# manuelbb-upb/Morbit.jl

Hardware: AMD Instinct MI355X
Metric: RBF build+solve+eval cycles/sec (higher is better)
Workload: dtype f64

## Files before the change

### morbit.jl_amd/csrc/common.hpp

```cpp
#pragma once
#include <hip/hip_runtime.h>
#include <rocblas/rocblas.h>
#include <rocsolver/rocsolver.h>

#include <cmath>
#include <cstdlib>
#include <cstdint>
#include <cstdio>
#include <cstring>
#include <map>
#include <string>
#include <vector>

#include "../../include/mrbf.h"
#include "descent_problem.hpp"
#include "model_pool.hpp"

namespace mrbf {

struct KP {
    int kid;
    double a, b;
    double a2;
    double sgn;
// ... 154 lines not shown
int input_fetch(mrbf_ctx *ctx, const double *src, size_t count, double *dst);
int input_view(mrbf_ctx *ctx, const double *user, size_t count, double *&arena, const double **dev);
int output_put(mrbf_ctx *ctx, double *dst, const double *src, size_t count);
int fetch_linear_rows(mrbf_ctx *ctx, const mrbf_ps_problem *prob, int d, double *A, double *b);
descent::Shape descent_shape(const mrbf_ps_problem *prob, const mrbf_model *const *models, int64_t n_starts,
                             std::vector<descent::SlotShape> &slots);
void pin_reset(mrbf_ctx *ctx);
void pin_flush(mrbf_ctx *ctx);
void pin_discard(mrbf_ctx *ctx);
char *pin_take(mrbf_ctx *ctx, size_t bytes);
struct PinGuard {
    mrbf_ctx *ctx;
    bool flushed = false;
    explicit PinGuard(mrbf_ctx *c) : ctx(c) { pin_reset(c); }
    void flush() {
        pin_flush(ctx);
        flushed = true;
    }
    ~PinGuard() {
        if (!flushed) pin_discard(ctx);
    }
    PinGuard(const PinGuard &) = delete;
    PinGuard &operator=(const PinGuard &) = delete;
};
enum HpinSlot : int {
    HPIN_FIT_FLAGS = 0,
    HPIN_FIT_SCAL = 4,
    HPIN_SMALL_FLAGS = 8,
    HPIN_SMALL_SCAL = 12,
    HPIN_SMALL_CHK = 16,
    HPIN_RESIDUAL = 20,
    HPIN_R4_COUNT = 24,
    HPIN_MEGA_STAT = 63,
};

inline int64_t round_up(int64_t x, int64_t m) { return (x + m - 1) / m * m; }

inline const char *mrbf_env(const char *name) {
    const char *gate = std::getenv("MRBF_EXPERIMENTS");
    if (!gate || std::atoi(gate) == 0) return nullptr;
    return std::getenv(name);
}

int launch_center_pad(mrbf_ctx *ctx, const double *X, int64_t n, int d, const double *mean_or_null, double *mean_out,
                      double *Xc, int64_t npad, int dpad, double *sq);
int launch_poly_matrix(mrbf_ctx *ctx, const double *C, int64_t n, int d, int q, double *Pi, int64_t ldpi);
int launch_transpose(mrbf_ctx *ctx, const double *in, int64_t rows, int64_t cols, double *out);
int launch_gram(mrbf_ctx *ctx, int mode, const double *C, const double *Xc, const double *sq, int64_t n, int64_t npad,
                int d, int dpad, const KP &kp, double *Phi, int64_t ld);
int launch_cross_gram(mrbf_ctx *ctx, const double *X, int64_t m, const double *C, int64_t n, int d, const KP &kp, double *K);
bool gram_w_applies(const mrbf_ctx *ctx, const mrbf_model *M);
int launch_gram_w(mrbf_ctx *ctx, const mrbf_model *M, double *Phi, int64_t ld, double **Wpart_out, double **rspart_out, int *nseg_out);
int launch_projection_small(mrbf_ctx *ctx, const mrbf_model *M, const double *Wpart, const double *rspart, int nseg, const double *linv,
                            const double *Q1, double *W1, double *G, double *scal, int *flags, int K2, int skip, double *PA, double *PB,
                            double *v0);
int eval_model(mrbf_ctx *ctx, const mrbf_model *M, int64_t m, const double *Xdev, double *vals_dev, double *jac_dev,
               mrbf_eval_info *info, EvalHints hints = {});
int potrf_blocked_tall(mrbf_ctx *ctx, int64_t ncols, int64_t mrows, double *A, int64_t lda, int *dinfo, double *linv_all, PotrfOpts opt = {});
int potrf_mega_tall(mrbf_ctx *ctx, int64_t ncols, int64_t mrows, double *A, int64_t lda, int *dinfo, double *linv_all, PotrfOpts opt = {});
mega::Knobs mega_knobs_from_env();
int potrf_lower(mrbf_ctx *ctx, int impl, int64_t n, double *A, int64_t lda, int *info_host);
int fit_model(mrbf_ctx *ctx, mrbf_model *M, const double *Ydev, mrbf_fit_info *info);
int build_model_shell(mrbf_ctx *ctx, int64_t n, int d, int k, const double *Cdev, int kid, double a, double b, int deg,
                      mrbf_model **out);
void destroy_model(mrbf_ctx *ctx, mrbf_model *M);
void model_set_dims(mrbf_model *M, int64_t n, int d, int k, int kid, double a, double b, int deg);
size_t model_block_layout(const mrbf_model *M, size_t off[7]);
void model_carve(mrbf_model *M, char *base, const size_t off[7]);
int model_block_acquire(mrbf_ctx *ctx, size_t total, void **p, size_t *bytes);
void model_block_release(mrbf_ctx *ctx, void *p, size_t bytes, bool slab = false);
int fit_check(mrbf_ctx *ctx, mrbf_model *M, const double *Y, mrbf_fit_info *info);
int mega_collect_stat(mrbf_ctx *ctx);
int mega_stat_enqueue(mrbf_ctx *ctx);
int mega_stat_finish(mrbf_ctx *ctx);

}
```

### morbit.jl_amd/csrc/gram_fused.hip

```cpp
#include "radial.hpp"

namespace mrbf {

typedef double v4d __attribute__((ext_vector_type(4)));
typedef double v2d __attribute__((ext_vector_type(2)));

constexpr int GW_LDT = 66;

template <int KID, bool FAST>
__global__ __launch_bounds__(256, 2) void gram_w_kernel(const double *__restrict__ Xc, const double *__restrict__ sq, int64_t n,
                                                        int64_t npad, double *__restrict__ Phi, int64_t ld, KP p, int nt, int nseg,
                                                        int seglen, double *__restrict__ Wpart, double *__restrict__ rspart, int dbg) {
    __shared__ __attribute__((aligned(16))) double T[2][64 * GW_LDT];
    __shared__ double Tsq[2][64];
    const int tid = threadIdx.x, lane = tid & 63, wave = tid >> 6;
    const int l15 = lane & 15, l4 = lane >> 4;
    const int seg = blockIdx.x % nseg, I = nt - 1 - (int)(blockIdx.x / nseg);
    const int jt0 = seg * seglen;
    const int jt1 = (jt0 + seglen < nt) ? jt0 + seglen : nt;
    const int64_t iw0 = (int64_t)I * 128 + 32 * wave;
    double bI[2][16];
#pragma unroll
    for (int it = 0; it < 2; ++it)
#pragma unroll
// ... 146 lines not shown
        }
    }
#pragma unroll
    for (int tt = 0; tt < 4; ++tt)
#pragma unroll
        for (int r = 0; r < 4; ++r) {
            const int t = tt * 16 + l4 + 4 * r;
#pragma unroll
            for (int it = 0; it < 2; ++it) Wpart[((int64_t)seg * 64 + t) * npad + iw0 + it * 16 + l15] = wacc[tt][it][r];
        }
#pragma unroll
    for (int it = 0; it < 2; ++it) {
        double x = rs[it];
        x += __shfl_xor(x, 16);
        x += __shfl_xor(x, 32);
        if (l4 == 0) rspart[(int64_t)seg * npad + iw0 + it * 16 + l15] = x;
    }
}

__device__ __forceinline__ double sum_partials(const double *__restrict__ p, int cnt, int64_t stride) {
    double sp[8] = {0.0, 0.0, 0.0, 0.0, 0.0, 0.0, 0.0, 0.0};
    int c = 0;
    for (; c + 32 <= cnt; c += 32) {
        double v[32];
#pragma unroll
        for (int u = 0; u < 32; ++u) v[u] = p[(int64_t)(c + u) * stride];
#pragma unroll
        for (int u = 0; u < 32; ++u) sp[u & 7] += v[u];
    }
    for (; c + 8 <= cnt; c += 8) {
        double v[8];
#pragma unroll
        for (int u = 0; u < 8; ++u) v[u] = p[(int64_t)(c + u) * stride];
#pragma unroll
        for (int u = 0; u < 8; ++u) sp[u] += v[u];
    }
    for (int u = 0; c + u < cnt; ++u) sp[u] += p[(int64_t)(c + u) * stride];
    return ((sp[0] + sp[1]) + (sp[2] + sp[3])) + ((sp[4] + sp[5]) + (sp[6] + sp[7]));
}

constexpr int PJ_LS = 68;
constexpr int PJ_QP = 80;

__device__ __forceinline__ v4d pj_tile(const double *As, const double *Bs, int mt, int nt, int K, int l15, int l4) {
    v4d acc = {0.0, 0.0, 0.0, 0.0};
    const double *ap = As + (mt * 16 + l15) * PJ_LS + l4;
    const double *bp = Bs + (nt * 16 + l15) * PJ_LS + l4;
    for (int k = 0; k < K; k += 4) acc = __builtin_amdgcn_mfma_f64_16x16x4f64(ap[k], bp[k], acc, 0, 0, 0);
    return acc;
}

__global__ __launch_bounds__(256) void proj_reduce_kernel(const double *__restrict__ Wpart, const double *__restrict__ rspart, int nseg,
                                                          int64_t npad, int64_t n, int d, int q, const double *__restrict__ linv,
                                                          const double *__restrict__ Q1, double rsqrtn, double *__restrict__ W1,
                                                          double *__restrict__ Gp, double *__restrict__ trp) {
    __shared__ double Ws[64 * PJ_LS];
    __shared__ double Ls[64 * PJ_LS];
    __shared__ double W1s[PJ_QP * PJ_LS];
    __shared__ double Qs[PJ_QP * PJ_LS];
    const int tid = threadIdx.x, i = tid & 63, g = tid >> 6;
    const int lane = tid & 63, wave = tid >> 6, l15 = lane & 15, l4 = lane >> 4;
    const int64_t R0 = (int64_t)blockIdx.x * 64;
    const bool live = R0 + i < n;
    constexpr int Q4 = PJ_QP / 4;
    double qv[Q4];
#pragma unroll
    for (int u = 0; u < Q4; ++u) {
        const int a = g + 4 * u;
        qv[u] = (a < q && live) ? Q1[R0 + i + (int64_t)a * npad] : 0.0;
    }
    const double rsv = (g == 0 && live) ? sum_partials(rspart + R0 + i, nseg, npad) * rsqrtn : 0.0;
    if (q > 1) {
        double lv[16];
#pragma unroll
        for (int u = 0; u < 16; ++u) {
            const int e = tid + 256 * u, c = e & 63, t = e >> 6;
            lv[u] = (c < d && t <= c) ? linv[c + (int64_t)t * 128] : 0.0;
        }
#pragma unroll
        for (int half = 0; half < 2; ++half) {
            double sv[8] = {0.0, 0.0, 0.0, 0.0, 0.0, 0.0, 0.0, 0.0};
            for (int s0 = 0; s0 < nseg; s0 += 8) {
                double wv[8][8];
#pragma unroll
                for (int u = 0; u < 8; ++u)
#pragma unroll
                    for (int sgm = 0; sgm < 8; ++sgm) {
                        const int t = g * 16 + half * 8 + u;
                        wv[u][sgm] = s0 + sgm < nseg ? Wpart[((int64_t)(s0 + sgm) * 64 + t) * npad + R0 + i] : 0.0;
                    }
#pragma unroll
                for (int u = 0; u < 8; ++u)
                    sv[u] += ((wv[u][0] + wv[u][1]) + (wv[u][2] + wv[u][3])) + ((wv[u][4] + wv[u][5]) + (wv[u][6] + wv[u][7]));
            }
#pragma unroll
            for (int u = 0; u < 8; ++u) Ws[i * PJ_LS + (g * 16 + half * 8 + u)] = live ? sv[u] : 0.0;
        }
#pragma unroll
        for (int u = 0; u < 16; ++u) {
            const int e = tid + 256 * u;
            Ls[(e & 63) * PJ_LS + (e >> 6)] = lv[u];
        }
    }
#pragma unroll
    for (int u = 0; u < Q4; ++u) {
        const int a = g + 4 * u;
        Qs[a * PJ_LS + i] = qv[u];
        if (a > d || q == 1) W1s[a * PJ_LS + i] = 0.0;
    }
    if (g == 0) {
        W1s[i] = rsv;
        W1[R0 + i] = rsv;
    }
    __syncthreads();
    if (q > 1) {
#pragma unroll 1
        for (int tile = wave; tile < 16; tile += 4) {
            const int ct = tile >> 2, it = tile & 3;
            const v4d acc = pj_tile(Ls, Ws, ct, it, 64, l15, l4);
#pragma unroll
            for (int r = 0; r < 4; ++r) {
                const int c = ct * 16 + l4 + 4 * r, ii = it * 16 + l15;
                if (c < d) {
                    W1s[(1 + c) * PJ_LS + ii] = acc[r];
                    W1[R0 + ii + (int64_t)(1 + c) * npad] = acc[r];
                }
            }
        }
    }
    __syncthreads();
    double *out = Gp + (size_t)blockIdx.x * q * q;
    const int qt = (q + 15) >> 4;
#pragma unroll 1
    for (int tile = wave; tile < qt * qt; tile += 4) {
        const int at = tile % qt, bt = tile / qt;
        const v4d acc = pj_tile(Qs, W1s, at, bt, 64, l15, l4);
#pragma unroll
        for (int r = 0; r < 4; ++r) {
            const int a = at * 16 + l4 + 4 * r, bb = bt * 16 + l15;
            if (a < q && bb < q) out[a + bb * q] = acc[r];
            if (at == bt && a == bb && a < q) Ls[a] = acc[r];
        }
    }
    __syncthreads();
    if (tid == 0) {
        double tr = 0.0;
        for (int a = 0; a < q; ++a) tr += Ls[a];
        trp[blockIdx.x] = tr;
    }
}

__global__ __launch_bounds__(256) void proj_shift_kernel(const double *__restrict__ Gp, const double *__restrict__ trp, int nchunks, int q,
                                                         double nphi0, double nmq, double *__restrict__ G, double *__restrict__ Mh,
                                                         double *__restrict__ scal, int *__restrict__ flags) {
    __shared__ double dg[256];
    __shared__ double smu;
    const int tid = threadIdx.x;
    const size_t qq = (size_t)q * q;
    const int idx = blockIdx.x * 256 + tid;
    const double *p0 = Gp + (idx < (int)qq ? idx : 0);
    double tv = 0.0;
    for (int c = tid; c < nchunks; c += 256) tv += trp[c];
    double s0[8] = {0, 0, 0, 0, 0, 0, 0, 0};
    int c = 0;
    for (; c + 64 <= nchunks; c += 64) {
        double v0[64];
#pragma unroll
        for (int u = 0; u < 64; ++u) v0[u] = p0[(size_t)(c + u) * qq];
#pragma unroll
        for (int u = 0; u < 64; ++u) s0[u & 7] += v0[u];
    }
    for (; c < nchunks; ++c) s0[c & 7] += p0[(size_t)c * qq];
    const double gv = ((s0[0] + s0[1]) + (s0[2] + s0[3])) + ((s0[4] + s0[5]) + (s0[6] + s0[7]));
    dg[tid] = tv;
    __syncthreads();
    for (int w = 128; w > 0; w >>= 1) {
        if (tid < w) dg[tid] += dg[tid + w];
        __syncthreads();
    }
    if (tid == 0) {
        const double tr = dg[0];
        const double mu = (nphi0 - tr) / nmq;
        const bool ok = mu > 0.0 && mu < 1e300;
        smu = ok ? mu : 1.0;
        if (blockIdx.x == 0) {
            scal[0] = tr;
            scal[1] = smu;
            flags[2] = ok ? 0 : 1;
        }
    }
    __syncthreads();
    if (idx < (int)qq) {
        G[idx] = gv;
        Mh[idx] = 0.5 * gv + ((idx % q) == (idx / q) ? 0.5 * smu : 0.0);
    }
}

__global__ __launch_bounds__(256) void proj_panels_kernel(const double *__restrict__ Q1, const double *__restrict__ W1,
                                                          const double *__restrict__ Mh, int64_t n, int64_t npad, int q, int K2, int skip,
                                                          double *__restrict__ PA, double *__restrict__ PB, double *__restrict__ v0) {
    __shared__ double Qs[64 * PJ_LS];
    __shared__ double Ms[PJ_QP * PJ_LS];
    const int tid = threadIdx.x, i = tid & 63, g = tid >> 6;
    const int lane = tid & 63, wave = tid >> 6, l15 = lane & 15, l4 = lane >> 4;
    const int64_t R0 = (int64_t)blockIdx.x * 64;
    const bool live = R0 + i < n;
    constexpr int QA = 17;
    double qv[QA];
#pragma unroll
    for (int u = 0; u < QA; ++u) {
        const int a = g + 4 * u;
        qv[u] = (a < q && live) ? Q1[R0 + i + (int64_t)a * npad] : 0.0;
    }
    constexpr int ME = (PJ_QP * PJ_LS + 255) / 256;
    double mv[ME];
#pragma unroll
    for (int u = 0; u < ME; ++u) {
        const int e = tid + 256 * u, bb = e / PJ_LS, a = e % PJ_LS;
        mv[u] = (a < q && bb < q) ? Mh[a + bb * q] : 0.0;
    }
#pragma unroll
    for (int u = 0; u < ME; ++u) {
        const int e = tid + 256 * u;
        if (e < PJ_QP * PJ_LS) Ms[e] = mv[u];
    }
#pragma unroll
    for (int u = 0; u < QA; ++u) Qs[i * PJ_LS + g + 4 * u] = qv[u];
    __syncthreads();
    const int qq = q - skip, qt = (q + 15) >> 4, K = (q + 3) & ~3;
#pragma unroll 1
    for (int tile = wave; tile < qt * 4; tile += 4) {
        const int bt = tile >> 2, it = tile & 3;
        const v4d acc = pj_tile(Ms, Qs, bt, it, K, l15, l4);
        const int ii = it * 16 + l15;
        const bool lv = R0 + ii < n;
        double w1[4], qb[4];
#pragma unroll
        for (int r = 0; r < 4; ++r) {
            const int b = bt * 16 + l4 + 4 * r;
            w1[r] = (b < q && lv) ? W1[R0 + ii + (int64_t)b * npad] : 0.0;
            qb[r] = b < q ? Qs[ii * PJ_LS + b] : 0.0;
        }
#pragma unroll
        for (int r = 0; r < 4; ++r) {
            const int b = bt * 16 + l4 + 4 * r;
            if (b >= q) continue;
            const double v = lv ? w1[r] - acc[r] : 0.0;
            if (b >= skip) {
                const int c = b - skip;
                PA[R0 + ii + (int64_t)c * npad] = qb[r];
                PB[R0 + ii + (int64_t)c * npad] = v;
                PA[R0 + ii + (int64_t)(qq + c) * npad] = v;
                PB[R0 + ii + (int64_t)(qq + c) * npad] = qb[r];
            } else {
                v0[R0 + ii] = v;
            }
        }
    }
    for (int c = 2 * qq + g; c < K2; c += 4) {
        PA[R0 + i + (int64_t)c * npad] = 0.0;
        PB[R0 + i + (int64_t)c * npad] = 0.0;
    }
}

bool gram_w_applies(const mrbf_ctx *ctx, const mrbf_model *M) {
    static const int on = mrbf_env("MRBF_GRAM_FUSED") ? atoi(mrbf_env("MRBF_GRAM_FUSED")) : 1;
    if (!on || ctx->gram_mode != 0) return false;
    if (M->dpad != 64 || M->q < 1 || M->q > 65 || M->n < 1024) return false;
    return M->kp.fast || M->kp.kid == MRBF_GAUSSIAN || M->kp.kid == MRBF_THIN_PLATE_SPLINE;
}

int launch_gram_w(mrbf_ctx *ctx, const mrbf_model *M, double *Phi, int64_t ld, double **Wpart_out, double **rspart_out, int *nseg_out) {
    const int nt = (int)(M->npad / 128);
    static const int dbg = mrbf_env("MRBF_GW_DBG") ? atoi(mrbf_env("MRBF_GW_DBG")) : 0;
    static const int wgs = mrbf_env("MRBF_GW_WGS") ? atoi(mrbf_env("MRBF_GW_WGS")) : 512;
    int nseg = wgs / nt;
    if (nseg < 1) nseg = 1;
    if (nseg > nt) nseg = nt;
    const int seglen = (nt + nseg - 1) / nseg;
    nseg = (nt + seglen - 1) / seglen;
    double *Wpart, *rspart;
    MRBF_TRY(get_buf(ctx, S_GW_PART, (size_t)nseg * 64 * M->npad, &Wpart));
    MRBF_TRY(get_buf(ctx, S_GW_RS, (size_t)nseg * M->npad, &rspart));
    const dim3 grid((unsigned)(nt * nseg));
    if (M->kp.fast) {
        MRBF_DISPATCH_KID(M->kp.kid, hipLaunchKernelGGL((gram_w_kernel<KID, true>), grid, dim3(256), 0, ctx->stream, M->Xc, M->sq, M->n,
                                                        M->npad, Phi, ld, M->kp, nt, nseg, seglen, Wpart, rspart, dbg));
    } else if (M->kp.kid == MRBF_GAUSSIAN) {
        hipLaunchKernelGGL((gram_w_kernel<MRBF_GAUSSIAN, false>), grid, dim3(256), 0, ctx->stream, M->Xc, M->sq, M->n, M->npad, Phi, ld,
                           M->kp, nt, nseg, seglen, Wpart, rspart, dbg);
    } else {
        hipLaunchKernelGGL((gram_w_kernel<MRBF_THIN_PLATE_SPLINE, false>), grid, dim3(256), 0, ctx->stream, M->Xc, M->sq, M->n, M->npad,
                           Phi, ld, M->kp, nt, nseg, seglen, Wpart, rspart, dbg);
    }
    MRBF_HIP(ctx, hipGetLastError());
    *Wpart_out = Wpart;
    *rspart_out = rspart;
    *nseg_out = nseg;
    return 0;
}

int launch_projection_small(mrbf_ctx *ctx, const mrbf_model *M, const double *Wpart, const double *rspart, int nseg, const double *linv,
                            const double *Q1, double *W1, double *G, double *scal, int *flags, int K2, int skip, double *PA, double *PB,
                            double *v0) {
    const int64_t n = M->n, npad = M->npad;
    const int q = M->q, nch = (int)(npad / 64);
    double *Gp, *Mh;
    MRBF_TRY(get_buf(ctx, S_GW_GP, (size_t)nch * q * q + nch, &Gp));
    MRBF_TRY(get_buf(ctx, S_GW_M, (size_t)q * q, &Mh));
    double *trp = Gp + (size_t)nch * q * q;
    hipLaunchKernelGGL(proj_reduce_kernel, dim3((unsigned)nch), dim3(256), 0, ctx->stream, Wpart, rspart, nseg, npad, n, M->d, q, linv, Q1,
                       1.0 / std::sqrt((double)n), W1, Gp, trp);
    hipLaunchKernelGGL(proj_shift_kernel, dim3((unsigned)((q * q + 255) / 256)), dim3(256), 0, ctx->stream, Gp, trp, nch, q,
                       (double)n * M->kp.phi0, (double)std::max<int64_t>(n - q, 1), G, Mh, scal, flags);
    hipLaunchKernelGGL(proj_panels_kernel, dim3((unsigned)nch), dim3(256), 0, ctx->stream, Q1, W1, Mh, n, npad, q, K2, skip, PA, PB, v0);
    MRBF_HIP(ctx, hipGetLastError());
    return 0;
}

}
```

### morbit.jl_amd/csrc/small.hip

```cpp
#include "chol_diag_core.hpp"
#include "radial.hpp"
#include "small.hpp"

#include <utility>

namespace mrbf {
namespace smallfit {

typedef double v4d __attribute__((ext_vector_type(4)));

__device__ __forceinline__ double phi_rt(double s, const KP &p) {
    switch (p.kid) {
        case MRBF_CUBIC: return p.fast ? rbf_phi_t<MRBF_CUBIC, true>(s, p) : rbf_phi_t<MRBF_CUBIC, false>(s, p);
        case MRBF_INV_MULTIQUADRIC: return p.fast ? rbf_phi_t<MRBF_INV_MULTIQUADRIC, true>(s, p) : rbf_phi_t<MRBF_INV_MULTIQUADRIC, false>(s, p);
        case MRBF_MULTIQUADRIC: return p.fast ? rbf_phi_t<MRBF_MULTIQUADRIC, true>(s, p) : rbf_phi_t<MRBF_MULTIQUADRIC, false>(s, p);
        case MRBF_THIN_PLATE_SPLINE: return rbf_phi_t<MRBF_THIN_PLATE_SPLINE, false>(s, p);
        default: return rbf_phi_t<MRBF_GAUSSIAN, false>(s, p);
    }
}

typedef __attribute__((address_space(1))) double gdbl;
__device__ __forceinline__ void gst(double *p, double v) { *(gdbl *)p = v; }
__device__ __forceinline__ double gld(const double *p) { return *(const gdbl *)p; }

// ... 837 lines not shown
                b = gld(&t.Y[(int64_t)(R0 + i) * t.k + l]) - fma(t.rsn, gld(&t.T1[(int64_t)l * t.q]), (part4[0][i] + part4[1][i]) + (part4[2][i] + part4[3][i]));
            gst(&t.B[(R0 + i) + (int64_t)l * t.npad], b);
            if (t.rows_out) gst(&t.rows_out[(t.npad + l) + (int64_t)(R0 + i) * t.ld], b);
        }
    }
    if (t.rows_out)
        for (int e = tid; e < 64 * t.xt; e += 256) {
            const int l = e % t.xt, r = e / t.xt;
            if (l >= t.k) gst(&t.rows_out[(t.npad + l) + (int64_t)(R0 + r) * t.ld], 0.0);
        }
}

}

bool small_fit_applies(const mrbf_ctx *ctx, int64_t n, int d, int k, int q, int path) {
    static const int off = mrbf_env("MRBF_SMALL_FIT") ? atoi(mrbf_env("MRBF_SMALL_FIT")) == 0 : 0;
    if (off || ctx->chol_impl == 1 || ctx->gram_mode == 1) return false;
    return n >= 1 && n <= 512 && d >= 1 && d <= 128 && k >= 1 && k <= 16 && n > q && (path == MRBF_PATH_CHOL || path == MRBF_PATH_PROJ_CHOL);
}

int small_fit_cluster(const mrbf_ctx *ctx, int count) {
    static const int env = mrbf_env("MRBF_SMALL_NC") ? atoi(mrbf_env("MRBF_SMALL_NC")) : 0;
    if (env == 1 || ctx->small_nc == 1 || !ctx->small_cluster_ok) return 1;
    const int groups = (std::max(count, 1) + 7) / 8;
    int nc = 1;
    while (2 * nc <= smallfit::MAX_CLUSTER && 8 * groups * 2 * nc <= ctx->ncu) nc *= 2;
    if (env > 1) nc = std::min(env, smallfit::MAX_CLUSTER);
    int p2 = 1;
    while (2 * p2 <= nc) p2 *= 2;
    return p2;
}

int launch_small_fit(mrbf_ctx *ctx, const smallfit::Prob *host_probs, int count, const smallfit::Prob *dev_probs, int nc) {
    if (count <= 0) return 0;
    const unsigned grid = nc == 1 ? (unsigned)count : 8u * (unsigned)nc * (unsigned)((count + 7) / 8);
    hipLaunchKernelGGL(smallfit::small_fit_kernel, dim3(grid), dim3(256), 0, ctx->stream, host_probs[0],
                       (count == 1 && !dev_probs) ? (const smallfit::Prob *)nullptr : dev_probs, count, nc);
    MRBF_HIP(ctx, hipGetLastError());
    return 0;
}

int launch_small_means(mrbf_ctx *ctx, const smallfit::Prob *dev_probs, int count) {
    if (count <= 0) return 0;
    hipLaunchKernelGGL(smallfit::small_mean_kernel, dim3((unsigned)count), dim3(256), 0, ctx->stream, dev_probs, count);
    MRBF_HIP(ctx, hipGetLastError());
    return 0;
}

bool tail_basis_applies(const mrbf_model *M) {
    static const int on = mrbf_env("MRBF_TAILQ") ? atoi(mrbf_env("MRBF_TAILQ")) : 1;
    return on && M->dpad == 64 && M->d >= 1 && M->d <= 64 && M->q == M->d + 1 && M->k >= 1 && M->k <= 16 && M->npad % 64 == 0;
}
int launch_tail_basis(mrbf_ctx *ctx, const mrbf_model *M, const double *Y, double *scratch, double *LinvX, double *T1, double *Q1, double *B,
                      double *rows_out, int64_t ld, int xt, int *flags) {
    smallfit::TailQ t;
    t.Xc = M->Xc;
    t.Y = Y;
    t.n = (int)M->n;
    t.npad = (int)M->npad;
    t.d = M->d;
    t.dpad = M->dpad;
    t.q = M->q;
    t.k = M->k;
    const int n16 = (t.n + 15) & ~15;
    t.np = std::min(32, std::max(4, t.n / 128));
    t.rows = ((n16 + t.np - 1) / t.np + 15) & ~15;
    t.Gx = scratch;
    t.part = scratch + 128 * 128;
    t.LinvX = LinvX;
    t.T1 = T1;
    t.Q1 = Q1;
    t.B = B;
    t.rows_out = rows_out;
    t.ld = ld;
    t.xt = xt;
    t.flags = flags;
    t.rsn = 1.0 / std::sqrt((double)M->n);
    hipLaunchKernelGGL(smallfit::tailq_gram_kernel, dim3((unsigned)t.np), dim3(256), 0, ctx->stream, t);
    hipLaunchKernelGGL(smallfit::tailq_factor_kernel, dim3(1), dim3(256), 0, ctx->stream, t);
    hipLaunchKernelGGL(smallfit::tailq_q1_kernel, dim3((unsigned)(M->npad / 64)), dim3(256), 0, ctx->stream, t);
    MRBF_HIP(ctx, hipGetLastError());
    return 0;
}
size_t tail_basis_scratch_doubles() { return (size_t)128 * 128 + (size_t)32 * smallfit::TQ_PS; }

}
```

### morbit.jl_amd/csrc/small.hpp

```cpp
#pragma once
#include "common.hpp"

namespace mrbf {
namespace smallfit {

struct Prob {
    int n, d, k, q, deg;
    int n16, npad, dpad, q16;
    KP kp;
    const double *C, *Y;
    double *Xc, *sq, *mean, *W, *Wc, *lam;
    double *ws;
    int *flags;
    double *scal;
    long long *stamps;
    int *cl;
    int mean_given;
    unsigned long long spin_ticks;
    int fault;
    int diag6;
};

constexpr int CL_WORDS = 24;
constexpr int MAX_CLUSTER = 16;
// ... 28 lines not shown
    c.T2 = take((size_t)c.ldz * 16);
    c.Z = take((size_t)c.ldz * 16 + 16);
    c.total = o;
    return c;
}

}

struct EvalDesc {
    const double *X;
    const double *mean;
    double *Xq, *xsq;
    const double *Cc, *csq, *Wc, *lam;
    int64_t npad, mpad, m;
    int d, k, q, tiles_per_split, nsplit;
    int ntiles;
    int nsub;
    KP kp;
    double *vpart, *sapart, *gpart;
    double *vals, *jac;
};
inline void eval_desc_model(EvalDesc &E, const mrbf_model *M, int64_t m, int nsplit) {
    E.mean = M->mean;
    E.Cc = M->Xc;
    E.csq = M->sq;
    E.Wc = M->Wc;
    E.lam = M->lam;
    E.npad = M->npad;
    E.d = M->d;
    E.k = M->k;
    E.q = M->q;
    E.kp = M->kp;
    E.m = m;
    E.mpad = round_up(m, 64);
    E.nsplit = nsplit;
    E.ntiles = (int)((M->n + 63) / 64);
    E.nsub = (int)((M->n + 15) / 16);
    E.tiles_per_split = (E.ntiles + nsplit - 1) / nsplit;
}
int eval_nsplit(const mrbf_ctx *ctx, int64_t m, int ntiles, bool check_call = false, bool population = false);
int outputs_per_pass(int k, int D, bool want_jac = true);
int eval_fused_batch(mrbf_ctx *ctx, const KP &kp, int D, int k, bool want_jac, const EvalDesc *host_descs, const EvalDesc *dev_descs, int count,
                     bool centred = false);
int center_pad_batch(mrbf_ctx *ctx, const EvalDesc *dev_descs, int count, int64_t max_mpad);

bool small_fit_applies(const mrbf_ctx *ctx, int64_t n, int d, int k, int q, int path);
int launch_small_fit(mrbf_ctx *ctx, const smallfit::Prob *host_probs, int count, const smallfit::Prob *dev_probs, int nc);
int small_fit_cluster(const mrbf_ctx *ctx, int count);
int launch_small_means(mrbf_ctx *ctx, const smallfit::Prob *dev_probs, int count);

bool tail_basis_applies(const mrbf_model *M);
size_t tail_basis_scratch_doubles();
int launch_tail_basis(mrbf_ctx *ctx, const mrbf_model *M, const double *Y, double *scratch, double *LinvX, double *T1, double *Q1, double *B,
                      double *rows_out, int64_t ld, int xt, int *flags);

}
```

### morbit.jl_amd/csrc/solve.hip

```cpp
#include "common.hpp"
#include "small.hpp"

namespace mrbf {

__global__ void fit_publish_kernel(const int *__restrict__ dinfo, const double *__restrict__ scal, const unsigned long long *__restrict__ dstat,
                                   int *__restrict__ hflags, double *__restrict__ hscal, unsigned long long *__restrict__ hstat) {
    const int t = threadIdx.x;
    if (t < 4) hflags[t] = dinfo[t];
    if (t >= 4 && t < 6 && scal) hscal[t - 4] = scal[t - 4];
    if (t == 6 && dstat && hstat) hstat[0] = dstat[0];
}

__global__ void fill_saddle_kernel(const double *__restrict__ Pi, int64_t n, int q, double *__restrict__ S, int64_t N) {
    const int64_t idx = (int64_t)blockIdx.x * blockDim.x + threadIdx.x;
    const int64_t tot = n * q;
    if (idx < tot) {
        const int64_t i = idx % n;
        const int t = (int)(idx / n);
        const double v = Pi[idx];
        S[i + (n + t) * N] = v;
        S[(n + t) + i * N] = v;
    } else if (idx < tot + (int64_t)q * q) {
        const int64_t r = idx - tot;
        S[(n + r % q) + (n + r / q) * N] = 0.0;
// ... 535 lines not shown
                                                         double *__restrict__ lam) {
    __shared__ double part4[4][64];
    const int tid = threadIdx.x, r = tid & 63, g = tid >> 6;
    const int64_t row = (int64_t)blockIdx.x * 64 + r;
    for (int l = 0; l < k; ++l) {
        double s0 = 0.0, s1 = 0.0;
        if (row < n) {
            int t = g;
            for (; t + 4 < q; t += 8) {
                s0 = fma(Q1[row + (int64_t)t * ldq], T2[t + (int64_t)l * q], s0);
                s1 = fma(Q1[row + (int64_t)(t + 4) * ldq], T2[t + 4 + (int64_t)l * q], s1);
            }
            if (t < q) s0 = fma(Q1[row + (int64_t)t * ldq], T2[t + (int64_t)l * q], s0);
        }
        __syncthreads();
        part4[g][r] = s0 + s1;
        __syncthreads();
        if (g == 0 && row < npad) {
            const double v = row < n ? Bw[row + (int64_t)l * ldb] - ((part4[0][r] + part4[1][r]) + (part4[2][r] + part4[3][r])) : 0.0;
            Wc[row + (int64_t)l * npad] = v;
            if (row < n) W[row * k + l] = v;
        }
    }
    if (blockIdx.x == 0)
        for (int e = tid; e < q * k; e += 256) lam[(int64_t)(e % q) * k + e / q] = lamsrc[(e % q) + (int64_t)(e / q) * q];
}

static int fit_chol(mrbf_ctx *ctx, mrbf_model *M, const double *Y, mrbf_fit_info *info, int *not_pd, int *gave_up, int impl = 0) {
    const int64_t n = M->n, npad = M->npad;
    const int k = M->k, q = M->q, d = M->d;
    const double one = 1.0, mhalf = -0.5;
    *not_pd = 0;
    *gave_up = 0;
    if (impl == 0) impl = ctx->chol_impl;
    const bool builtin = impl != 1;
    PotrfOpts popt;
    popt.impl = impl;
    const int xt = builtin ? (int)round_up(k, 128) : 0;
    const int64_t ld = npad + xt;
    double *Phi, *B;
    int *dinfo;
    MRBF_TRY(get_buf(ctx, S_PHI, (size_t)ld * npad, &Phi));
    MRBF_TRY(get_buf(ctx, S_RHS, (size_t)npad * k, &B));
    MRBF_TRY(get_buf(ctx, S_INFO, (size_t)4, &dinfo));
    MRBF_HIP(ctx, hipMemsetAsync(dinfo, 0, 4 * sizeof(int), ctx->stream));
    const bool tailq = q > 1 && tail_basis_applies(M) && M->k == k;
    if (!tailq) hipLaunchKernelGGL(rhs_from_values_kernel, dim3(nblk(npad * k)), dim3(256), 0, ctx->stream, Y, n, k, B, npad);
    double *Q1 = nullptr, *Wm = nullptr, *G = nullptr, *T1 = nullptr, *scal = nullptr, *Tall = nullptr, *LxInv = nullptr;
    int64_t lt = 0, dq = 0;
    info->mu = 0.0;
    hipStream_t main_stream = ctx->stream;
    const bool side = q > 0 && ctx->panel_stream && ctx->panel_stream != main_stream && n >= 2048;
    const bool fused = q > 0 && gram_w_applies(ctx, M) && (q == 1 || round_up(d, 128) == 128);
    if (q > 0) {
        MRBF_TRY(get_buf(ctx, S_Q1, (size_t)npad * q, &Q1));
        MRBF_TRY(get_buf(ctx, S_W1, (size_t)npad * q, &Wm));
        MRBF_TRY(get_buf(ctx, S_G, (size_t)q * q, &G));
        MRBF_TRY(get_buf(ctx, S_T1, (size_t)q * k, &T1));
        MRBF_TRY(get_buf(ctx, S_MISC, (size_t)8, &scal));
        if (side) {
            MRBF_HIP(ctx, hipEventRecord(ctx->evx[0], main_stream));
            MRBF_HIP(ctx, hipStreamWaitEvent(ctx->panel_stream, ctx->evx[0], 0));
            ctx->stream = ctx->panel_stream;
        }
        struct RestoreStream {
            mrbf_ctx *c;
            hipStream_t s;
            ~RestoreStream() { c->stream = s; }
        } restore{ctx, main_stream};
        if (tailq) {
            double *scratch;
            MRBF_TRY(get_buf(ctx, S_PI, tail_basis_scratch_doubles(), &scratch));
            MRBF_TRY(get_buf(ctx, S_QR_INV, (size_t)128 * 128, &LxInv));
            MRBF_TRY(launch_tail_basis(ctx, M, Y, scratch, LxInv, T1, Q1, B, builtin ? Phi : nullptr, ld, xt, dinfo));
        } else if (q > 1) {
            dq = round_up(d, 128);
            lt = dq + npad;
            MRBF_TRY(get_buf(ctx, S_PI, (size_t)lt * dq, &Tall));
            MRBF_HIP(ctx, hipMemsetAsync(Tall, 0, (size_t)lt * dq * sizeof(double), ctx->stream));
            hipLaunchKernelGGL(xc_to_tall_kernel, dim3(nblk(n * d)), dim3(256), 0, ctx->stream, M->Xc, n, d, M->dpad, Tall, lt, dq);
            MRBF_TRY(tsmm_tn(ctx, n, d, d, 1.0, Tall + dq, lt, Tall + dq, lt, 0.0, Tall, lt));
            MRBF_TRY(launch_pad_identity(ctx, Tall, d, dq, lt));
            if (dq == 128) MRBF_TRY(get_buf(ctx, S_QR_INV, (size_t)128 * 128, &LxInv));
            MRBF_TRY(potrf_blocked_tall(ctx, dq, lt, Tall, lt, dinfo + 1, LxInv, popt));
        }
        if (!tailq) hipLaunchKernelGGL(build_q1_kernel, dim3(nblk(npad * q)), dim3(256), 0, ctx->stream, Tall, lt, dq, n, npad, q, Q1);
        if (!fused) MRBF_HIP(ctx, hipMemsetAsync(Wm, 0, (size_t)npad * q * sizeof(double), ctx->stream));
        if (!tailq) {
            MRBF_TRY(tsmm_tn(ctx, n, q, k, 1.0, Q1, npad, B, npad, 0.0, T1, q));
            hipLaunchKernelGGL(sub_qt_kernel, dim3((unsigned)((n + 63) / 64)), dim3(256), 0, ctx->stream, B, npad, Q1, npad, T1, n, q, k);
            if (builtin) hipLaunchKernelGGL(set_rhs_rows_kernel, dim3(nblk(npad * xt)), dim3(256), 0, ctx->stream, Phi, ld, npad, xt, B, k);
        }
        if (side) MRBF_HIP(ctx, hipEventRecord(ctx->evx[1], ctx->stream));
    }
    ctx->stream = main_stream;
    MRBF_HIP(ctx, hipEventRecord(ctx->ev[0], ctx->stream));
    double *Wpart = nullptr, *rspart = nullptr;
    int nseg = 0;
    if (fused)
        MRBF_TRY(launch_gram_w(ctx, M, Phi, ld, &Wpart, &rspart, &nseg));
    else
        MRBF_TRY(launch_gram(ctx, ctx->gram_mode, M->C, M->Xc, M->sq, n, M->npad, M->d, M->dpad, M->kp, Phi, ld));
    MRBF_HIP(ctx, hipEventRecord(ctx->ev[1], ctx->stream));
    if (side) MRBF_HIP(ctx, hipStreamWaitEvent(ctx->stream, ctx->evx[1], 0));
    if (fused) {
        const int skip = (q > 1 && round_up(2 * (q - 1), 16) < round_up(2 * q, 16)) ? 1 : 0;
        const int K2 = (int)round_up(2 * (q - skip), 16);
        double *PA, *PB, *v0 = nullptr;
        MRBF_TRY(get_buf(ctx, S_STAGE_C, (size_t)npad * K2, &PA));
        MRBF_TRY(get_buf(ctx, S_STAGE_D, (size_t)npad * K2, &PB));
        if (skip) MRBF_TRY(get_buf(ctx, S_V0, (size_t)npad, &v0));
        MRBF_TRY(launch_projection_small(ctx, M, Wpart, rspart, nseg, LxInv, Q1, Wm, G, scal, dinfo, K2, skip, PA, PB, v0));
        MRBF_TRY(launch_update_lower(ctx, PA, npad, PB, npad, Phi, ld, npad / 128, K2, v0, 1.0 / std::sqrt((double)n), n));
    } else if (q > 0) {
        MRBF_TRY(symm_panel(ctx, n, npad, q, Phi, ld, Q1, npad, Wm, npad, true, 1.0 / std::sqrt((double)n)));
        MRBF_TRY(tsmm_tn(ctx, n, q, q, 1.0, Q1, npad, Wm, npad, 0.0, G, q));
        hipLaunchKernelGGL(trace_kernel, dim3(1), dim3(256), 0, ctx->stream, G, q, scal);
        MRBF_BLAS(ctx, rocblas_dgemm(ctx->blas, rocblas_operation_none, rocblas_operation_none, (int)n, q, q, &mhalf, Q1, (int)npad,
                                     G, q, &one, Wm, (int)npad));
        hipLaunchKernelGGL(shift_from_trace_kernel, dim3(1), dim3(1), 0, ctx->stream, scal, (double)n * M->kp.phi0,
                           (double)std::max<int64_t>(n - q, 1), dinfo);
        const int skip = (q > 1 && round_up(2 * (q - 1), 16) < round_up(2 * q, 16)) ? 1 : 0;
        const int K2 = (int)round_up(2 * (q - skip), 16);
        double *PA, *PB, *v0 = nullptr;
        MRBF_TRY(get_buf(ctx, S_STAGE_C, (size_t)npad * K2, &PA));
        MRBF_TRY(get_buf(ctx, S_STAGE_D, (size_t)npad * K2, &PB));
        if (skip) MRBF_TRY(get_buf(ctx, S_V0, (size_t)npad, &v0));
        hipLaunchKernelGGL(build_panels_kernel, dim3(nblk(npad * K2)), dim3(256), 0, ctx->stream, Q1, Wm, scal, n, npad, q, K2, skip, PA, PB, v0);
        MRBF_TRY(launch_update_lower(ctx, PA, npad, PB, npad, Phi, ld, npad / 128, K2, v0, 1.0 / std::sqrt((double)n), n));
    }
    MRBF_HIP(ctx, hipEventRecord(ctx->ev[2], ctx->stream));
    int hinfo = 0;
    double *linv_all = nullptr;
    if (builtin) {
        MRBF_TRY(get_buf(ctx, S_CHOL_WS, (size_t)npad * 128, &linv_all));
        MRBF_TRY(launch_pad_identity(ctx, Phi, n, npad, ld));
        if (q == 0) hipLaunchKernelGGL(set_rhs_rows_kernel, dim3(nblk(npad * xt)), dim3(256), 0, ctx->stream, Phi, ld, npad, xt, B, k);
        popt.xreal = k;
        popt.info_clean = true;
        MRBF_TRY(potrf_blocked_tall(ctx, npad, npad + xt, Phi, ld, dinfo, linv_all, popt));
        MRBF_HIP(ctx, hipEventRecord(ctx->ev[3], ctx->stream));
    } else {
        int *dpot;
        MRBF_TRY(get_buf(ctx, S_IPIV, (size_t)4, &dpot));
        MRBF_BLAS(ctx, rocsolver_dpotrf(ctx->blas, rocblas_fill_lower, (int)n, Phi, (int)ld, dpot));
        MRBF_HIP(ctx, hipMemcpyAsync(dinfo, dpot, sizeof(int), hipMemcpyDeviceToDevice, ctx->stream));
        MRBF_HIP(ctx, hipEventRecord(ctx->ev[3], ctx->stream));
    }
    double *T1w = nullptr;
    if (q > 0) MRBF_TRY(get_buf(ctx, S_T1W, (size_t)q * k, &T1w));
    auto solve_tail = [&](bool persistent) -> int {
        if (builtin) {
            hipLaunchKernelGGL(get_rhs_rows_kernel, dim3(nblk(npad * k)), dim3(256), 0, ctx->stream, Phi, ld, npad, B, k);
            if (persistent)
                MRBF_TRY(backsolve_persistent(ctx, npad, Phi, ld, linv_all, B, npad, k, dinfo + 3));
            else
                MRBF_TRY(backsolve_blocked(ctx, npad, Phi, ld, linv_all, B, npad, k));
        } else {
            MRBF_BLAS(ctx, rocsolver_dpotrs(ctx->blas, rocblas_fill_lower, (int)n, k, Phi, (int)ld, B, (int)npad));
        }
        static const int tail3 = mrbf_env("MRBF_TAIL3") ? atoi(mrbf_env("MRBF_TAIL3")) : 1;
        if (tail3 && q > 0 && q <= 129 && k <= 16 && (q == 1 || LxInv)) {
            const int nch = (int)(npad / 64);
            double *T2, *part;
            MRBF_TRY(get_buf(ctx, S_T2, (size_t)q * k, &T2));
            MRBF_TRY(get_buf(ctx, S_TAIL_PART, (size_t)nch * 2 * k * q, &part));
            hipLaunchKernelGGL(tail_dots_kernel, dim3((unsigned)nch), dim3(256), 0, ctx->stream, B, npad, Q1, Wm, npad, n, q, k, part);
            hipLaunchKernelGGL(tail_coeff_kernel, dim3(1), dim3(1024), 0, ctx->stream, part, nch, q, k, q > 1 ? d : 0, T1, G, fused ? 1.0 : 0.5, LxInv,
                               std::sqrt((double)n), M->mean, T2, T1w);
            hipLaunchKernelGGL(tail_apply_kernel, dim3((unsigned)nch), dim3(256), 0, ctx->stream, B, npad, Q1, npad, T2, T1w, n, M->npad, q, k, M->W,
                               M->Wc, M->lam);
            MRBF_HIP(ctx, hipGetLastError());
            return 0;
        }
        if (q > 0) {
            double *T2;
            MRBF_TRY(get_buf(ctx, S_T2, (size_t)q * k, &T2));
            MRBF_HIP(ctx, hipMemcpyAsync(T1w, T1, (size_t)q * k * sizeof(double), hipMemcpyDeviceToDevice, ctx->stream));
            MRBF_TRY(tsmm_tn(ctx, n, q, k, 1.0, Q1, npad, B, npad, 0.0, T2, q));
            hipLaunchKernelGGL(sub_qt_kernel, dim3((unsigned)((n + 63) / 64)), dim3(256), 0, ctx->stream, B, npad, Q1, npad, T2, n, q, k);
            MRBF_TRY(tsmm_tn(ctx, n, q, k, -1.0, Wm, npad, B, npad, 1.0, T1w, q));
            if (q > 1) {
                if (LxInv)
                    hipLaunchKernelGGL(apply_linv_t_kernel, dim3(1), dim3(256), 0, ctx->stream, LxInv, d, T1w + 1, (int64_t)q, k);
// ... 304 lines not shown
```

Before: 176.4.

## Recompute Q1 from Xc and Linv in projection kernels to relax side-stream dependency

```diff
diff --git a/morbit.jl_amd/csrc/common.hpp b/morbit.jl_amd/csrc/common.hpp
--- a/morbit.jl_amd/csrc/common.hpp
+++ b/morbit.jl_amd/csrc/common.hpp
@@ -230,7 +230,7 @@
 bool gram_w_applies(const mrbf_ctx *ctx, const mrbf_model *M);
 int launch_gram_w(mrbf_ctx *ctx, const mrbf_model *M, double *Phi, int64_t ld, double **Wpart_out, double **rspart_out, int *nseg_out);
 int launch_projection_small(mrbf_ctx *ctx, const mrbf_model *M, const double *Wpart, const double *rspart, int nseg, const double *linv,
-                            const double *Q1, double *W1, double *G, double *scal, int *flags, int K2, int skip, double *PA, double *PB,
+                            double *W1, double *G, double *scal, int *flags, int K2, int skip, double *PA, double *PB,
                             double *v0);
 int eval_model(mrbf_ctx *ctx, const mrbf_model *M, int64_t m, const double *Xdev, double *vals_dev, double *jac_dev,
                mrbf_eval_info *info, EvalHints hints = {});
diff --git a/morbit.jl_amd/csrc/gram_fused.hip b/morbit.jl_amd/csrc/gram_fused.hip
--- a/morbit.jl_amd/csrc/gram_fused.hip
+++ b/morbit.jl_amd/csrc/gram_fused.hip
@@ -222,22 +222,22 @@
 
 __global__ __launch_bounds__(256) void proj_reduce_kernel(const double *__restrict__ Wpart, const double *__restrict__ rspart, int nseg,
                                                           int64_t npad, int64_t n, int d, int q, const double *__restrict__ linv,
-                                                          const double *__restrict__ Q1, double rsqrtn, double *__restrict__ W1,
+                                                          const double *__restrict__ Xc, double rsqrtn, double *__restrict__ W1,
                                                           double *__restrict__ Gp, double *__restrict__ trp) {
     __shared__ double Ws[64 * PJ_LS];
     __shared__ double Ls[64 * PJ_LS];
     __shared__ double W1s[PJ_QP * PJ_LS];
     __shared__ double Qs[PJ_QP * PJ_LS];
+    double *Xs = W1s;
     const int tid = threadIdx.x, i = tid & 63, g = tid >> 6;
     const int lane = tid & 63, wave = tid >> 6, l15 = lane & 15, l4 = lane >> 4;
     const int64_t R0 = (int64_t)blockIdx.x * 64;
     const bool live = R0 + i < n;
     constexpr int Q4 = PJ_QP / 4;
-    double qv[Q4];
-#pragma unroll
-    for (int u = 0; u < Q4; ++u) {
-        const int a = g + 4 * u;
-        qv[u] = (a < q && live) ? Q1[R0 + i + (int64_t)a * npad] : 0.0;
+    double xv[16];
+    if (q > 1) {
+#pragma unroll
+        for (int u = 0; u < 16; ++u) xv[u] = Xc[R0 * 64 + tid + 256 * u];
     }
     const double rsv = (g == 0 && live) ? sum_partials(rspart + R0 + i, nseg, npad) * rsqrtn : 0.0;
     if (q > 1) {
@@ -271,29 +271,50 @@
             const int e = tid + 256 * u;
             Ls[(e & 63) * PJ_LS + (e >> 6)] = lv[u];
         }
+#pragma unroll
+        for (int u = 0; u < 16; ++u) {
+            const int e = tid + 256 * u;
+            Xs[(e >> 6) * PJ_LS + (e & 63)] = xv[u];
+        }
     }
 #pragma unroll
     for (int u = 0; u < Q4; ++u) {
         const int a = g + 4 * u;
-        Qs[a * PJ_LS + i] = qv[u];
+        Qs[a * PJ_LS + i] = (a == 0 && live) ? rsqrtn : 0.0;
+    }
+    if (g == 0) W1[R0 + i] = rsv;
+    __syncthreads();
+    v4d wx[4];
+    if (q > 1) {
+#pragma unroll
+        for (int v = 0; v < 4; ++v) {
+            const int tile = wave + 4 * v, ct = tile >> 2, it = tile & 3;
+            const v4d qa = pj_tile(Ls, Xs, ct, it, 64, l15, l4);
+            wx[v] = pj_tile(Ls, Ws, ct, it, 64, l15, l4);
+#pragma unroll
+            for (int r = 0; r < 4; ++r) {
+                const int c = ct * 16 + l4 + 4 * r, ii = it * 16 + l15;
+                if (c < d) Qs[(1 + c) * PJ_LS + ii] = R0 + ii < n ? qa[r] : 0.0;
+            }
+        }
+    }
+    __syncthreads();
+#pragma unroll
+    for (int u = 0; u < Q4; ++u) {
+        const int a = g + 4 * u;
         if (a > d || q == 1) W1s[a * PJ_LS + i] = 0.0;
     }
-    if (g == 0) {
-        W1s[i] = rsv;
-        W1[R0 + i] = rsv;
-    }
-    __syncthreads();
-    if (q > 1) {
-#pragma unroll 1
-        for (int tile = wave; tile < 16; tile += 4) {
-            const int ct = tile >> 2, it = tile & 3;
-            const v4d acc = pj_tile(Ls, Ws, ct, it, 64, l15, l4);
+    if (g == 0) W1s[i] = rsv;
+    if (q > 1) {
+#pragma unroll
+        for (int v = 0; v < 4; ++v) {
+            const int tile = wave + 4 * v, ct = tile >> 2, it = tile & 3;
 #pragma unroll
             for (int r = 0; r < 4; ++r) {
                 const int c = ct * 16 + l4 + 4 * r, ii = it * 16 + l15;
                 if (c < d) {
-                    W1s[(1 + c) * PJ_LS + ii] = acc[r];
-                    W1[R0 + ii + (int64_t)(1 + c) * npad] = acc[r];
+                    W1s[(1 + c) * PJ_LS + ii] = wx[v][r];
+                    W1[R0 + ii + (int64_t)(1 + c) * npad] = wx[v][r];
                 }
             }
         }
@@ -366,21 +387,28 @@
     }
 }
 
-__global__ __launch_bounds__(256) void proj_panels_kernel(const double *__restrict__ Q1, const double *__restrict__ W1,
+__global__ __launch_bounds__(256) void proj_panels_kernel(const double *__restrict__ Xc, const double *__restrict__ linv, int d,
+                                                          double rsqrtn, const double *__restrict__ W1,
                                                           const double *__restrict__ Mh, int64_t n, int64_t npad, int q, int K2, int skip,
                                                           double *__restrict__ PA, double *__restrict__ PB, double *__restrict__ v0) {
     __shared__ double Qs[64 * PJ_LS];
     __shared__ double Ms[PJ_QP * PJ_LS];
+    __shared__ double Ls[64 * PJ_LS];
+    __shared__ double Xs[64 * PJ_LS];
     const int tid = threadIdx.x, i = tid & 63, g = tid >> 6;
     const int lane = tid & 63, wave = tid >> 6, l15 = lane & 15, l4 = lane >> 4;
     const int64_t R0 = (int64_t)blockIdx.x * 64;
     const bool live = R0 + i < n;
     constexpr int QA = 17;
-    double qv[QA];
-#pragma unroll
-    for (int u = 0; u < QA; ++u) {
-        const int a = g + 4 * u;
-        qv[u] = (a < q && live) ? Q1[R0 + i + (int64_t)a * npad] : 0.0;
+    double xv[16], lv[16];
+    if (q > 1) {
+#pragma unroll
+        for (int u = 0; u < 16; ++u) xv[u] = Xc[R0 * 64 + tid + 256 * u];
+#pragma unroll
+        for (int u = 0; u < 16; ++u) {
+            const int e = tid + 256 * u, c = e & 63, t = e >> 6;
+            lv[u] = (c < d && t <= c) ? linv[c + (int64_t)t * 128] : 0.0;
+        }
     }
     constexpr int ME = (PJ_QP * PJ_LS + 255) / 256;
     double mv[ME];
@@ -395,8 +423,29 @@
         if (e < PJ_QP * PJ_LS) Ms[e] = mv[u];
     }
 #pragma unroll
-    for (int u = 0; u < QA; ++u) Qs[i * PJ_LS + g + 4 * u] = qv[u];
-    __syncthreads();
+    for (int u = 0; u < QA; ++u) Qs[i * PJ_LS + g + 4 * u] = (g + 4 * u == 0 && live) ? rsqrtn : 0.0;
+    if (q > 1) {
+#pragma unroll
+        for (int u = 0; u < 16; ++u) {
+            const int e = tid + 256 * u;
+            Ls[(e & 63) * PJ_LS + (e >> 6)] = lv[u];
+            Xs[(e >> 6) * PJ_LS + (e & 63)] = xv[u];
+        }
+    }
+    __syncthreads();
+    if (q > 1) {
+#pragma unroll
+        for (int v = 0; v < 4; ++v) {
+            const int tile = wave + 4 * v, ct = tile >> 2, it = tile & 3;
+            const v4d qa = pj_tile(Ls, Xs, ct, it, 64, l15, l4);
+#pragma unroll
+            for (int r = 0; r < 4; ++r) {
+                const int c = ct * 16 + l4 + 4 * r, ii = it * 16 + l15;
+                if (c < d) Qs[ii * PJ_LS + 1 + c] = R0 + ii < n ? qa[r] : 0.0;
+            }
+        }
+        __syncthreads();
+    }
     const int qq = q - skip, qt = (q + 15) >> 4, K = (q + 3) & ~3;
 #pragma unroll 1
     for (int tile = wave; tile < qt * 4; tile += 4) {
@@ -471,7 +520,7 @@
 }
 
 int launch_projection_small(mrbf_ctx *ctx, const mrbf_model *M, const double *Wpart, const double *rspart, int nseg, const double *linv,
-                            const double *Q1, double *W1, double *G, double *scal, int *flags, int K2, int skip, double *PA, double *PB,
+                            double *W1, double *G, double *scal, int *flags, int K2, int skip, double *PA, double *PB,
                             double *v0) {
     const int64_t n = M->n, npad = M->npad;
     const int q = M->q, nch = (int)(npad / 64);
@@ -479,11 +528,12 @@
     MRBF_TRY(get_buf(ctx, S_GW_GP, (size_t)nch * q * q + nch, &Gp));
     MRBF_TRY(get_buf(ctx, S_GW_M, (size_t)q * q, &Mh));
     double *trp = Gp + (size_t)nch * q * q;
-    hipLaunchKernelGGL(proj_reduce_kernel, dim3((unsigned)nch), dim3(256), 0, ctx->stream, Wpart, rspart, nseg, npad, n, M->d, q, linv, Q1,
-                       1.0 / std::sqrt((double)n), W1, Gp, trp);
+    const double rsqrtn = 1.0 / std::sqrt((double)n);
+    hipLaunchKernelGGL(proj_reduce_kernel, dim3((unsigned)nch), dim3(256), 0, ctx->stream, Wpart, rspart, nseg, npad, n, M->d, q, linv, M->Xc,
+                       rsqrtn, W1, Gp, trp);
     hipLaunchKernelGGL(proj_shift_kernel, dim3((unsigned)((q * q + 255) / 256)), dim3(256), 0, ctx->stream, Gp, trp, nch, q,
                        (double)n * M->kp.phi0, (double)std::max<int64_t>(n - q, 1), G, Mh, scal, flags);
-    hipLaunchKernelGGL(proj_panels_kernel, dim3((unsigned)nch), dim3(256), 0, ctx->stream, Q1, W1, Mh, n, npad, q, K2, skip, PA, PB, v0);
+    hipLaunchKernelGGL(proj_panels_kernel, dim3((unsigned)nch), dim3(256), 0, ctx->stream, M->Xc, linv, M->d, rsqrtn, W1, Mh, n, npad, q, K2, skip, PA, PB, v0);
     MRBF_HIP(ctx, hipGetLastError());
     return 0;
 }
diff --git a/morbit.jl_amd/csrc/small.hip b/morbit.jl_amd/csrc/small.hip
--- a/morbit.jl_amd/csrc/small.hip
+++ b/morbit.jl_amd/csrc/small.hip
@@ -913,7 +913,7 @@
     return on && M->dpad == 64 && M->d >= 1 && M->d <= 64 && M->q == M->d + 1 && M->k >= 1 && M->k <= 16 && M->npad % 64 == 0;
 }
 int launch_tail_basis(mrbf_ctx *ctx, const mrbf_model *M, const double *Y, double *scratch, double *LinvX, double *T1, double *Q1, double *B,
-                      double *rows_out, int64_t ld, int xt, int *flags) {
+                      double *rows_out, int64_t ld, int xt, int *flags, hipEvent_t ev_linv) {
     smallfit::TailQ t;
     t.Xc = M->Xc;
     t.Y = Y;
@@ -939,6 +939,7 @@
     t.rsn = 1.0 / std::sqrt((double)M->n);
     hipLaunchKernelGGL(smallfit::tailq_gram_kernel, dim3((unsigned)t.np), dim3(256), 0, ctx->stream, t);
     hipLaunchKernelGGL(smallfit::tailq_factor_kernel, dim3(1), dim3(256), 0, ctx->stream, t);
+    if (ev_linv) MRBF_HIP(ctx, hipEventRecord(ev_linv, ctx->stream));
     hipLaunchKernelGGL(smallfit::tailq_q1_kernel, dim3((unsigned)(M->npad / 64)), dim3(256), 0, ctx->stream, t);
     MRBF_HIP(ctx, hipGetLastError());
     return 0;
diff --git a/morbit.jl_amd/csrc/small.hpp b/morbit.jl_amd/csrc/small.hpp
--- a/morbit.jl_amd/csrc/small.hpp
+++ b/morbit.jl_amd/csrc/small.hpp
@@ -104,6 +104,6 @@
 bool tail_basis_applies(const mrbf_model *M);
 size_t tail_basis_scratch_doubles();
 int launch_tail_basis(mrbf_ctx *ctx, const mrbf_model *M, const double *Y, double *scratch, double *LinvX, double *T1, double *Q1, double *B,
-                      double *rows_out, int64_t ld, int xt, int *flags);
+                      double *rows_out, int64_t ld, int xt, int *flags, hipEvent_t ev_linv = nullptr);
 
 }
diff --git a/morbit.jl_amd/csrc/solve.hip b/morbit.jl_amd/csrc/solve.hip
--- a/morbit.jl_amd/csrc/solve.hip
+++ b/morbit.jl_amd/csrc/solve.hip
@@ -611,6 +611,7 @@
     hipStream_t main_stream = ctx->stream;
     const bool side = q > 0 && ctx->panel_stream && ctx->panel_stream != main_stream && n >= 2048;
     const bool fused = q > 0 && gram_w_applies(ctx, M) && (q == 1 || round_up(d, 128) == 128);
+    const bool split = side && fused && (tailq || q == 1);
     if (q > 0) {
         MRBF_TRY(get_buf(ctx, S_Q1, (size_t)npad * q, &Q1));
         MRBF_TRY(get_buf(ctx, S_W1, (size_t)npad * q, &Wm));
@@ -631,7 +632,7 @@
             double *scratch;
             MRBF_TRY(get_buf(ctx, S_PI, tail_basis_scratch_doubles(), &scratch));
             MRBF_TRY(get_buf(ctx, S_QR_INV, (size_t)128 * 128, &LxInv));
-            MRBF_TRY(launch_tail_basis(ctx, M, Y, scratch, LxInv, T1, Q1, B, builtin ? Phi : nullptr, ld, xt, dinfo));
+            MRBF_TRY(launch_tail_basis(ctx, M, Y, scratch, LxInv, T1, Q1, B, builtin ? Phi : nullptr, ld, xt, dinfo, split ? ctx->evx[1] : nullptr));
         } else if (q > 1) {
             dq = round_up(d, 128);
             lt = dq + npad;
@@ -650,7 +651,7 @@
             hipLaunchKernelGGL(sub_qt_kernel, dim3((unsigned)((n + 63) / 64)), dim3(256), 0, ctx->stream, B, npad, Q1, npad, T1, n, q, k);
             if (builtin) hipLaunchKernelGGL(set_rhs_rows_kernel, dim3(nblk(npad * xt)), dim3(256), 0, ctx->stream, Phi, ld, npad, xt, B, k);
         }
-        if (side) MRBF_HIP(ctx, hipEventRecord(ctx->evx[1], ctx->stream));
+        if (side) MRBF_HIP(ctx, hipEventRecord(ctx->evx[split ? 2 : 1], ctx->stream));
     }
     ctx->stream = main_stream;
     MRBF_HIP(ctx, hipEventRecord(ctx->ev[0], ctx->stream));
@@ -661,7 +662,7 @@
     else
         MRBF_TRY(launch_gram(ctx, ctx->gram_mode, M->C, M->Xc, M->sq, n, M->npad, M->d, M->dpad, M->kp, Phi, ld));
     MRBF_HIP(ctx, hipEventRecord(ctx->ev[1], ctx->stream));
-    if (side) MRBF_HIP(ctx, hipStreamWaitEvent(ctx->stream, ctx->evx[1], 0));
+    if (side && (!split || tailq)) MRBF_HIP(ctx, hipStreamWaitEvent(ctx->stream, ctx->evx[1], 0));
     if (fused) {
         const int skip = (q > 1 && round_up(2 * (q - 1), 16) < round_up(2 * q, 16)) ? 1 : 0;
         const int K2 = (int)round_up(2 * (q - skip), 16);
@@ -669,7 +670,7 @@
         MRBF_TRY(get_buf(ctx, S_STAGE_C, (size_t)npad * K2, &PA));
         MRBF_TRY(get_buf(ctx, S_STAGE_D, (size_t)npad * K2, &PB));
         if (skip) MRBF_TRY(get_buf(ctx, S_V0, (size_t)npad, &v0));
-        MRBF_TRY(launch_projection_small(ctx, M, Wpart, rspart, nseg, LxInv, Q1, Wm, G, scal, dinfo, K2, skip, PA, PB, v0));
+        MRBF_TRY(launch_projection_small(ctx, M, Wpart, rspart, nseg, LxInv, Wm, G, scal, dinfo, K2, skip, PA, PB, v0));
         MRBF_TRY(launch_update_lower(ctx, PA, npad, PB, npad, Phi, ld, npad / 128, K2, v0, 1.0 / std::sqrt((double)n), n));
     } else if (q > 0) {
         MRBF_TRY(symm_panel(ctx, n, npad, q, Phi, ld, Q1, npad, Wm, npad, true, 1.0 / std::sqrt((double)n)));
@@ -689,6 +690,7 @@
         MRBF_TRY(launch_update_lower(ctx, PA, npad, PB, npad, Phi, ld, npad / 128, K2, v0, 1.0 / std::sqrt((double)n), n));
     }
     MRBF_HIP(ctx, hipEventRecord(ctx->ev[2], ctx->stream));
+    if (split) MRBF_HIP(ctx, hipStreamWaitEvent(ctx->stream, ctx->evx[2], 0));
     int hinfo = 0;
     double *linv_all = nullptr;
     if (builtin) {
```

New measurement: 176.7, median of 4. Within noise of the previous version (+0.1%).
